# clysto/tinyimgcodec

Hardware: AMD Instinct MI355X
Metric: Mpixels/s encode (DCT+quant kernel) (higher is better)
Workload: dtype f32+f64

## Files before the change

tinyimgcodec_amd/csrc/lint_strip_kernel.py:

```python
#!/usr/bin/env python3
import os
import re
import shutil
import subprocess
import sys
import tempfile

LLVM = "/opt/rocm/lib/llvm/bin"


class ToolsMissing(RuntimeError):
    pass


def device_code_objects(lib_path, tmp):
    bundler, objdump, readelf = (os.path.join(LLVM, t) for t in ("clang-offload-bundler", "llvm-objdump", "llvm-readelf"))
    if shutil.which("objcopy") is None or not all(os.path.exists(t) for t in (bundler, objdump, readelf)):
        raise ToolsMissing("binutils / ROCm llvm tools not available")
    fat = os.path.join(tmp, "fat.bin")
    subprocess.run(["objcopy", "-O", "binary", "--only-section=.hip_fatbin", lib_path, fat], check=True)
    blob = open(fat, "rb").read()
    magic = b"__CLANG_OFFLOAD_BUNDLE__"
    starts = [i for i in range(len(blob)) if blob.startswith(magic, i)]
    out = []
    for k, st in enumerate(starts):
        part = os.path.join(tmp, "bundle%d.bin" % k)
        with open(part, "wb") as f:
            f.write(blob[st:starts[k + 1] if k + 1 < len(starts) else len(blob)])
        co = os.path.join(tmp, "dev%d.co" % k)
        subprocess.run([bundler, "--unbundle", "--type=o", "--input=" + part, "--targets=hipv4-amdgcn-amd-amdhsa--gfx950", "--output=" + co], check=True)
        out.append((co, objdump, readelf))
    return out


def check(lib_path):
    found = []
    with tempfile.TemporaryDirectory() as tmp:
        for co, objdump, readelf in device_code_objects(lib_path, tmp):
            dis = subprocess.run([objdump, "-d", "--no-show-raw-insn", co], capture_output=True, text=True, check=True).stdout
            for m in re.finditer(r"<(_ZN3tic17dctq_strip_kernel\w+)>:\n(.*?)(?=\n\n|\Z)", dis, re.S):
                name, body = m.group(1), m.group(2)
                insns = [ln.split("//")[0].strip() for ln in body.splitlines() if ln.strip()]
                reserved = re.compile(r"\bv7[2-9]\b|\bv\[(\d+):(\d+)\]")

                def touches(ins):
                    for mm in reserved.finditer(ins):
                        if mm.group(1) is None:
                            return True
                        if int(mm.group(2)) >= 72 and int(mm.group(1)) <= 79:
                            return True
                    return False

                n_loads = n_moves = n_take = n_cvt = 0
                for k, ins in enumerate(insns):
                    if not touches(ins):
                        continue
                    if re.match(r"global_load_dwordx2 v\[7[246]:7[357]\], v\d+, s\[\d+:\d+\]", ins) or re.match(r"global_load_dwordx4 v\[76:79\], v\d+, s\[\d+:\d+\]", ins):
                        n_loads += 1
                        continue
                    tk = re.match(r"ds_write_b64 v(\d+), v\[7[246]:7[357]\]$", ins)
                    cv = re.match(r"v_cvt_f32_ubyte[0-3](_e32)? v(\d+), v(7[2-9])$", ins)
                    mv = re.match(r"v_mov_b32(_e32)? v(\d+), v(7[2-9])$", ins)
                    assert (tk and int(tk.group(1)) < 72) or (cv and int(cv.group(2)) < 72) or (mv and int(mv.group(2)) < 72), "unexpected use of a reserved register: " + ins
                    prev = insns[k - 1]
                    if tk:
                        n_take += 1
                        assert prev.startswith("s_waitcnt vmcnt("), "the LDS store out of a landing pair is not behind its counted wait: %s | %s" % (prev, ins)
                    elif cv:
                        n_cvt += 1
                        assert prev.startswith("s_waitcnt vmcnt(") or re.match(r"v_cvt_f32_ubyte[0-3](_e32)? v\d+, v7[2-9]$", prev), \
                            "a conversion out of a landing register is not behind its counted wait: %s | %s" % (prev, ins)
                    else:
                        n_moves += 1
                cols = n_take > 0
                assert n_loads >= 7 and n_moves >= 4 and ((cols and n_take >= 5 and n_cvt == 0) or (not cols and n_cvt >= 24 and n_cvt % 8 == 0)), (name, n_loads, n_take, n_cvt, n_moves)
                assert "accvgpr" not in body and "scratch_" not in body, "the strip kernel uses accumulator registers or scratch"
                notes = subprocess.run([readelf, "--notes", co], capture_output=True, text=True, check=True).stdout
                blk = [e for e in notes.split("\n  - .agpr_count:") if (".name:" in e and name in e)][0]
                blk = ".agpr_count:" + blk
                assert re.search(r"\.vgpr_count:\s+80\b", blk) and re.search(r"\.private_segment_fixed_size:\s+0\b", blk) and re.search(r"\.agpr_count:\s+0\b", blk), blk
                found.append("%s: 80 VGPRs, no AGPRs, no scratch; v72..v79 named by %d loads, %d %s, %d moves only"
                             % ("columns-first" if cols else "rows-first", n_loads, n_take if cols else n_cvt, "LDS stores" if cols else "conversions", n_moves))
    if len(found) == 2:
        return "dctq_strip_kernel | " + " | ".join(found)
    raise AssertionError("both instantiations of dctq_strip_kernel expected in %s, found %d" % (lib_path, len(found)))


if __name__ == "__main__":
    try:
        print("lint_strip_kernel: " + check(sys.argv[1]))
    except ToolsMissing as e:
        sys.stderr.write("lint_strip_kernel: %s\n" % e)
        sys.exit(2)
    except AssertionError as e:
        sys.stderr.write("lint_strip_kernel FAILED: %s\n" % (e,))
        sys.exit(1)
```

tinyimgcodec_amd/csrc/tic_kernels.hip:

```cpp
#include <hip/hip_runtime.h>
#include <hip/hip_ext.h>
#include <stddef.h>
#include <stdint.h>
#include <stdlib.h>
#include <string.h>
#include <type_traits>

#include "tic_hooks.h"
#include "tic_kernels.h"
#include "tic_rd_plan.h"
#include "tic_strip_plan.h"
#include "tic_math.h"

namespace tic {

#define TIC_DPP_QP_XOR1 0xB1
#define TIC_DPP_QP_XOR2 0x4E
#define TIC_DPP_ROW_SHL4 0x104
#define TIC_DPP_ROW_SHR4 0x114

__device__ __forceinline__ uint32_t perm_b32(uint32_t hi_src, uint32_t lo_src, uint32_t sel) {
    return __builtin_amdgcn_perm(hi_src, lo_src, sel);
}

__device__ __forceinline__ void transpose8x8_bytes(uint32_t &lo, uint32_t &hi, int i) {
    uint32_t nhi = (uint32_t)__builtin_amdgcn_update_dpp((int)hi, (int)lo, TIC_DPP_ROW_SHL4, 0xf, 0x5, false);
    uint32_t nlo = (uint32_t)__builtin_amdgcn_update_dpp((int)lo, (int)hi, TIC_DPP_ROW_SHR4, 0xf, 0xa, false);
    lo = nlo;
    hi = nhi;
    uint32_t selB = (i & 2) ? 0x03020706u : 0x05040100u;
    uint32_t plo = (uint32_t)__builtin_amdgcn_mov_dpp((int)lo, TIC_DPP_QP_XOR2, 0xf, 0xf, true);
    uint32_t phi = (uint32_t)__builtin_amdgcn_mov_dpp((int)hi, TIC_DPP_QP_XOR2, 0xf, 0xf, true);
    lo = perm_b32(plo, lo, selB);
    hi = perm_b32(phi, hi, selB);
    uint32_t selC = (i & 1) ? 0x03070105u : 0x06020400u;
    plo = (uint32_t)__builtin_amdgcn_mov_dpp((int)lo, TIC_DPP_QP_XOR1, 0xf, 0xf, true);
    phi = (uint32_t)__builtin_amdgcn_mov_dpp((int)hi, TIC_DPP_QP_XOR1, 0xf, 0xf, true);
    lo = perm_b32(plo, lo, selC);
    hi = perm_b32(phi, hi, selC);
}

__device__ __forceinline__ void transpose8x8_bytes_shfl(uint32_t &lo, uint32_t &hi, int i) {
    uint32_t row[2] = {lo, hi};
    uint32_t col_lo = 0, col_hi = 0;
    int base = (threadIdx.x & 63) & ~7;
    for (int r = 0; r < 8; r++) {
        uint32_t l = __shfl(row[0], base + r, 64), h = __shfl(row[1], base + r, 64);
        uint32_t w = (i < 4) ? l : h;
        uint32_t byte = (w >> (8 * (i & 3))) & 0xffu;
        if (r < 4)
            col_lo |= byte << (8 * r);
        else
            col_hi |= byte << (8 * (r - 4));
    }
    lo = col_lo;
    hi = col_hi;
}

__device__ __forceinline__ void wave_lds_fence() {
    __builtin_amdgcn_fence(__ATOMIC_RELEASE, "wavefront");
    __builtin_amdgcn_wave_barrier();
    __builtin_amdgcn_fence(__ATOMIC_ACQUIRE, "wavefront");
}

__device__ __forceinline__ int reflect_index(int i, int n) {
    if (i < n) return i;
    if (n >= 8) return 2 * (n - 1) - i;
    if (n == 1) return 0;
    int p = 2 * (n - 1), j = i;
    while (j >= p) j -= p;
    return j < n ? j : p - j;
}

constexpr int kWavesPerWG = 4;
static_assert(kWavesPerWG == kStripWavesPerWG, "tic_strip_plan.h plans for this workgroup");
constexpr int kLdsStrideDw = 68;
constexpr int kZzStrideB = 144;
constexpr int kLdsWaveBytes = 8 * kLdsStrideDw * 4;

struct Strip {
    int by, bx;
    bool valid;
    size_t oblk;
};

__device__ __forceinline__ void load_block_row(const uint8_t *__restrict__ img, int h, int w, long stride, bool aligned8,
                                               const Strip &s, int i, uint32_t &lo, uint32_t &hi) {
    lo = 0;
    hi = 0;
    if (!s.valid) return;
    int y = reflect_index(s.by * 8 + i, h);
    int x0 = s.bx * 8;
    const uint8_t *p = img + (long)y * stride + x0;
    if (aligned8 && x0 + 8 <= w) {
        uint2 v = *reinterpret_cast<const uint2 *>(p);
        lo = v.x;
        hi = v.y;
    } else {
        const uint8_t *rowp = img + (long)y * stride;
#pragma unroll
        for (int k = 0; k < 8; k++) {
            uint32_t b = rowp[reflect_index(x0 + k, w)];
            if (k < 4)
                lo |= b << (8 * k);
            else
                hi |= b << (8 * (k - 4));
        }
    }
}

__device__ __forceinline__ void transpose8x8_dwords(uint32_t *lds, int b, int i, uint32_t v[8]) {
    uint32_t *blk = lds + b * kLdsStrideDw;
#pragma unroll
    for (int u = 0; u < 8; u++) blk[u * 8 + i] = v[u];
    wave_lds_fence();
    const uint4 *rp = reinterpret_cast<const uint4 *>(blk + i * 8);
    uint4 a = rp[0], c = rp[1];
    v[0] = a.x; v[1] = a.y; v[2] = a.z; v[3] = a.w;
    v[4] = c.x; v[5] = c.y; v[6] = c.z; v[7] = c.w;
    wave_lds_fence();
}

__device__ __forceinline__ void exact_block(uint32_t colLo, uint32_t colHi, uint32_t *lds, int b, int i,
                                         const DctqConsts *__restrict__ C, int q[8]) {
    double c[8];
#pragma unroll
    for (int r = 0; r < 4; r++) {
        c[r] = (double)((int)((colLo >> (8 * r)) & 0xffu) - 128);
        c[r + 4] = (double)((int)((colHi >> (8 * r)) & 0xffu) - 128);
    }
    dct8_exact(c[0], c[1], c[2], c[3], c[4], c[5], c[6], c[7]);
    uint32_t w[8];
#pragma unroll
    for (int k = 0; k < 8; k++) w[k] = (uint32_t)__double2loint(c[k]);
    transpose8x8_dwords(lds, b, i, w);
    uint32_t wh[8];
#pragma unroll
    for (int k = 0; k < 8; k++) wh[k] = (uint32_t)__double2hiint(c[k]);
    transpose8x8_dwords(lds, b, i, wh);
#pragma unroll
    for (int k = 0; k < 8; k++) c[k] = __hiloint2double((int)wh[k], (int)w[k]);
    dct8_exact(c[0], c[1], c[2], c[3], c[4], c[5], c[6], c[7]);
    const double *div = C->div + i * 8;
#pragma unroll
    for (int v = 0; v < 8; v++) {
        q[v] = (int)rint(c[v] / div[v]);
        __builtin_amdgcn_sched_barrier(0);
    }
}

__device__ __forceinline__ void store_zigzag(uint32_t *lds, int b, int i, const uint16_t zz[8], const int q[8],
                                             int16_t *__restrict__ out, const Strip &s) {
    char *blk = reinterpret_cast<char *>(lds) + b * kZzStrideB;
#pragma unroll
    for (int v = 0; v < 8; v++) *reinterpret_cast<int16_t *>(blk + zz[v]) = (int16_t)q[v];
    wave_lds_fence();
    uint4 val = *reinterpret_cast<const uint4 *>(blk + i * 16);
    wave_lds_fence();
    if (s.valid) *reinterpret_cast<uint4 *>(out + s.oblk * 64 + i * 8) = val;
}

__device__ __forceinline__ Strip make_strip(int tile, int ntiles, int tiles_x, int bw, int b) {
    Strip s;
    int ty = tile / tiles_x;
    int tx = tile - ty * tiles_x;
    s.by = ty;
    s.bx = tx * 8 + b;
    s.valid = (tile < ntiles) && (s.bx < bw);
    s.oblk = (size_t)ty * bw + s.bx;
    return s;
}

__global__ __launch_bounds__(kWavesPerWG * 64) void dctq_exact_kernel(DctqArgs a) {
    __shared__ __attribute__((aligned(16))) uint32_t lds_all[kWavesPerWG][kLdsWaveBytes / 4];
    a.img += (long)blockIdx.y * a.frame_stride_in;
    a.out = reinterpret_cast<int16_t *>(reinterpret_cast<char *>(a.out) + (long)blockIdx.y * a.frame_stride_out);
    const int lane = threadIdx.x & 63, wave = threadIdx.x >> 6;
    const int b = lane >> 3, i = lane & 7;
    uint32_t *lds = lds_all[wave];
    int tile = blockIdx.x * kWavesPerWG + wave;
    int ntiles = a.ntiles;
    if (a.rem_mode) {
        const int bh = a.ntiles / a.tiles_x, rw = a.tiles_x - a.fast_tx;
        const int n_right = bh * rw, n_bottom = (bh - a.fast_ty) * a.fast_tx;
        ntiles = 0;
        if (tile < n_right) {
            tile = (tile / rw) * a.tiles_x + a.fast_tx + tile % rw;
            ntiles = a.ntiles;
        } else if (tile < n_right + n_bottom) {
            const int k = tile - n_right;
            tile = (a.fast_ty + k / a.fast_tx) * a.tiles_x + k % a.fast_tx;
            ntiles = a.ntiles;
        }
    }
    Strip s = make_strip(tile, ntiles, a.tiles_x, a.bw, b);
    uint32_t lo, hi;
    load_block_row(a.img, a.h, a.w, a.stride, a.aligned8, s, i, lo, hi);
    transpose8x8_bytes(lo, hi, i);
    int q[8];
    exact_block(lo, hi, lds, b, i, a.consts, q);
    const uint4 zzv = *reinterpret_cast<const uint4 *>(a.consts->zzofs + i * 8);
    uint16_t zz[8] = {(uint16_t)zzv.x, (uint16_t)(zzv.x >> 16), (uint16_t)zzv.y, (uint16_t)(zzv.y >> 16),
                      (uint16_t)zzv.z, (uint16_t)(zzv.z >> 16), (uint16_t)zzv.w, (uint16_t)(zzv.w >> 16)};
    store_zigzag(lds, b, i, zz, q, a.out, s);
}

constexpr int kTWaveBytes = kLdsWaveBytes;
constexpr int kTHalfDw = 272;
constexpr int kZzWaveBytes = 8 * kZzStrideB;
constexpr int kPxBlkBytes = 80;
constexpr int kChunkStrips = 8;

__device__ __forceinline__ void quant_fma(float z, float mul, uint32_t &bits, float &d) {
    const float s = fmaf(z, mul, kMagic);
    bits = __float_as_uint(s);
    const float nr = kMagic - s;
    d = fmaf(z, mul, nr);
}

__device__ __forceinline__ void store16_wt_nt(void *p, const uint4 &v) {
    typedef uint32_t u32x4 __attribute__((ext_vector_type(4)));
    const u32x4 d = {v.x, v.y, v.z, v.w};
    asm volatile("global_store_dwordx4 %0, %1, off sc1 nt" : : "v"(p), "v"(d) : "memory");
}
__device__ __forceinline__ void store16_wt_nt(const void *sbase, uint32_t voff, const uint4 &v) {
    typedef uint32_t u32x4 __attribute__((ext_vector_type(4)));
    const u32x4 d = {v.x, v.y, v.z, v.w};
    asm volatile("global_store_dwordx4 %0, %1, %2 sc1 nt" : : "v"(voff), "v"(d), "s"(sbase) : "memory");
}

constexpr int kBatch = 8;
constexpr int kBatchWaveBytes = kBatch * (128 + 64) + 64;

template <int CTRL>
__device__ __forceinline__ double dpp_f64(double x) {
    const int lo = __builtin_amdgcn_mov_dpp(__double2loint(x), CTRL, 0xf, 0xf, true);
    const int hi = __builtin_amdgcn_mov_dpp(__double2hiint(x), CTRL, 0xf, 0xf, true);
    return __hiloint2double(hi, lo);
}

__device__ __forceinline__ int rational_quad(const uint32_t *ldsT, int b, int i, const double *cst_rat) {
#pragma clang fp contract(off)
    const int w = i >> 2, k = i & 3;
    const uint32_t ca = (0x05010300u >> (8 * k)) & 0xffu, cb = (0x06020407u >> (8 * k)) & 0xffu;
    const uint32_t *row = ldsT + w * 128 + 4 * b;
    const float fa = __uint_as_float(row[(ca >> 2) * kTHalfDw + (ca & 3)]);
    const float fb = __uint_as_float(row[(cb >> 2) * kTHalfDw + (cb & 3)]);
    const double K = w ? (kTW3 * 0.5) : (kSq2h * 0.5);
    const double ya = (double)fa * K, yb = (double)fb * K;
    const double p = ya + yb;
    const double s2 = p + dpp_f64<TIC_DPP_QP_XOR1>(p);
    const double o = dpp_f64<TIC_DPP_QP_XOR2>(s2);
    const double E = (k & 1) ? s2 - o : s2 + o;
    const double X = E * ((k & 1) ? (kTW3 * 0.5) : (kSq2h * 0.5));
    const double div = cst_rat[2 * w + (k & 1)], rdiv = cst_rat[4 + 2 * w + (k & 1)];
    return (int)rint(div_rn(X, div, rdiv));
}

__device__ __forceinline__ int rational_slim(uint32_t rowLo, uint32_t rowHi, int i, const double *cst_rat) {
#pragma clang fp contract(off)
    uint32_t lo = perm_b32(rowHi, rowLo, 0x04030700u);
    uint32_t hi = perm_b32(rowHi, rowLo, 0x06050201u);
    transpose8x8_bytes(lo, hi, i);
    const uint32_t tot = __builtin_amdgcn_sad_u8(lo, 0u, __builtin_amdgcn_sad_u8(hi, 0u, 0u));
    const uint32_t sa = __builtin_amdgcn_sad_u8(lo & 0xff0000ffu, 0u, __builtin_amdgcn_sad_u8(hi & 0xff0000ffu, 0u, 0u));
    const int e0 = (int)tot - 1024, e4 = 2 * (int)sa - (int)tot;
    double y0 = (double)e0 * (kSq2h * 0.5);
    double y4 = (double)e4 * (kTW3 * 0.5);
    y0 = y0 + dpp_f64<TIC_DPP_QP_XOR1>(y0);
    y4 = y4 + dpp_f64<TIC_DPP_QP_XOR1>(y4);
    y0 = y0 + dpp_f64<TIC_DPP_QP_XOR2>(y0);
    y4 = y4 + dpp_f64<TIC_DPP_QP_XOR2>(y4);
    const double b0 = dpp_f64<TIC_DPP_ROW_SHL4>(y0), b4 = dpp_f64<TIC_DPP_ROW_SHL4>(y4);
    const double A = (i & 2) ? y4 : y0, B = (i & 2) ? b4 : b0;
    const double E = (i & 1) ? A - B : A + B;
    const double X = E * ((i & 1) ? (kTW3 * 0.5) : (kSq2h * 0.5));
    const double div = cst_rat[i & 3], rdiv = cst_rat[4 + (i & 3)];
    return (int)rint(div_rn(X, div, rdiv));
}
__device__ __forceinline__ unsigned long long wave_redo_block(const uint8_t *px , double *tbuf ,
                                                              const double *cosm, const double *rdiv, const uint16_t *zzofs, int16_t *img16,
                                                              int lane) {
    const int u = lane >> 3, c = lane & 7;
    typedef double d2 __attribute__((ext_vector_type(2)));
    const d2 *mu = reinterpret_cast<const d2 *>(cosm + u * 8), *mc = reinterpret_cast<const d2 *>(cosm + c * 8);
    const d2 m0 = mu[0], m1 = mu[1], m2 = mu[2], m3 = mu[3];
    double x[8];
#pragma unroll
    for (int r = 0; r < 8; r++) x[r] = (double)((int)px[r * 8 + c] - 128);
    double ta = m0.x * x[0], tb = m0.y * x[1];
    ta = fma(m1.x, x[2], ta); tb = fma(m1.y, x[3], tb);
    ta = fma(m2.x, x[4], ta); tb = fma(m2.y, x[5], tb);
    ta = fma(m3.x, x[6], ta); tb = fma(m3.y, x[7], tb);
    tbuf[u * 8 + c] = ta + tb;
    const d2 n0 = mc[0], n1 = mc[1], n2 = mc[2], n3 = mc[3];
    wave_lds_fence();
    const d2 *tu = reinterpret_cast<const d2 *>(tbuf + u * 8);
    const d2 y0 = tu[0], y1 = tu[1], y2 = tu[2], y3 = tu[3];
    double xa = n0.x * y0.x, xb = n0.y * y0.y;
    xa = fma(n1.x, y1.x, xa); xb = fma(n1.y, y1.y, xb);
    xa = fma(n2.x, y2.x, xa); xb = fma(n2.y, y2.y, xb);
    xa = fma(n3.x, y3.x, xa); xb = fma(n3.y, y3.y, xb);
    const double X = xa + xb;
    const double tq = X * rdiv[lane], rq = rint(tq);
    const bool rational = (lane & 0x1b) == 0;
    const bool decided = fabs(tq - rq) < 0.5 - 1e-9;
    if (decided && !rational) img16[zzofs[lane] >> 1] = (int16_t)(int)rq;
    const unsigned long long und = __ballot(!decided && !rational);
    wave_lds_fence();
    return und;
}

__device__ __forceinline__ uint32_t second_level_8(uint32_t colLo, uint32_t colHi, uint32_t *lds, int b, int i, const double *mul64, int q[8]) {
    double c[8];
#pragma unroll
    for (int r = 0; r < 4; r++) {
        c[r] = (double)(int)((colLo >> (8 * r)) & 0xffu);
        c[r + 4] = (double)(int)((colHi >> (8 * r)) & 0xffu);
    }
    dct8_aan(c[0], c[1], c[2], c[3], c[4], c[5], c[6], c[7]);
    c[0] -= 1024.0;
    uint32_t w[8], wh[8];
#pragma unroll
    for (int k = 0; k < 8; k++) w[k] = (uint32_t)__double2loint(c[k]);
    transpose8x8_dwords(lds, b, i, w);
#pragma unroll
    for (int k = 0; k < 8; k++) wh[k] = (uint32_t)__double2hiint(c[k]);
    transpose8x8_dwords(lds, b, i, wh);
#pragma unroll
    for (int k = 0; k < 8; k++) c[k] = __hiloint2double((int)wh[k], (int)w[k]);
    dct8_aan(c[0], c[1], c[2], c[3], c[4], c[5], c[6], c[7]);
    uint32_t und = 0;
#pragma unroll
    for (int v = 0; v < 8; v++) {
        const double t = c[v] * mul64[i * 8 + v], r = rint(t);
        q[v] = (int)r;
        if (!(fabs(t - r) < 0.5 - 1e-9)) und |= 1u << v;
    }
    return und;
}

struct StripKernargs {
    const uint8_t *img;
    const DctqConsts *consts;
    StripHead hd;
    StripWarm w;
    DctqArgs a;
};
static_assert(offsetof(StripKernargs, hd) == 16 && sizeof(StripHead) == 40 && offsetof(StripKernargs, w) == 64, "leading scalars, then one line");

template <class T>
__device__ __forceinline__ uint32_t lds_addr(T *p) {
    return (uint32_t)(uintptr_t)(__attribute__((address_space(3))) char *)(p);
}
template <class T>
__device__ __forceinline__ T *lds_ptr(uint32_t v) {
    return (T *)(__attribute__((address_space(3))) T *)(uintptr_t)v;
}

template <bool kCols>
__global__ __launch_bounds__(kWavesPerWG * 64, 6) __attribute__((amdgpu_num_vgpr(72))) void dctq_strip_kernel(
    const uint8_t *img, const DctqConsts *consts, unsigned long long hd_split, uint32_t hd_stride, uint32_t hd_misc, uint32_t hd_tstep,
    uint32_t hd_nfast, uint32_t hd_fast_tx, uint32_t hd_magic_fast_tx, uint32_t hd_in_step32, uint32_t hd_step_tx, StripWarm w, DctqArgs a) {
    const StripHead hd = {hd_split, hd_stride, hd_misc, hd_tstep, hd_nfast, hd_fast_tx, hd_magic_fast_tx, hd_in_step32, hd_step_tx};
    __shared__ __attribute__((aligned(16))) uint32_t ldsT_all[kWavesPerWG][kTWaveBytes / 4];
    __shared__ __attribute__((aligned(16))) uint32_t ldsZ_all[kWavesPerWG][kZzWaveBytes / 4];
    __shared__ __attribute__((aligned(16))) unsigned char cst_blk[kStripBlkBytes];
    __shared__ __attribute__((aligned(16))) uint32_t bat_all[kWavesPerWG][kBatchWaveBytes / 4];
    const int lane = threadIdx.x & 63;
    const int wave = __builtin_amdgcn_readfirstlane(threadIdx.x >> 6);
    uint32_t *ldsT = ldsT_all[wave];
    char *ldsZ = reinterpret_cast<char *>(ldsZ_all[wave]);
    const uint16_t *cst_zz = reinterpret_cast<const uint16_t *>(cst_blk + kBlkZz);
    const double *cst_rat = reinterpret_cast<const double *>(cst_blk + kBlkRat);
    uint4 *bat_img = reinterpret_cast<uint4 *>(bat_all[wave]);
    uint2 *bat_pix = reinterpret_cast<uint2 *>(bat_all[wave] + kBatch * 32);
    uint32_t *bat_id = bat_all[wave] + kBatch * 48;
    const DctqConsts *__restrict__ C = consts;
    const uint8_t *img_s = img;
    if (__builtin_expect(blockIdx.z != 0, 0)) {
        asm volatile("" : : : "memory");
        img_s += (long)blockIdx.z * w.frame_stride_in;
    }

    const int lr = lane >> 3, lb = lane & 7;
    const int b = lane >> 3, i = lane & 7;
    unsigned long long mask_exact = 0;
    uint32_t n_second = 0, n_quad = 0;
    int nE = 0;
    int t_first, n_my;
    int16_t *out_f;
    uint32_t st_off = (uint32_t)lane * 16u;
    {
        typedef float f32x4 __attribute__((ext_vector_type(4)));
        typedef uint32_t u32x4 __attribute__((ext_vector_type(4)));
        f32x4 m0, m1;
        f32x4 thr;
        u32x4 zzv;
        u32x4 c_fill;
        {
            constexpr int kPpw = kStripBlkPieces / kWavesPerWG;
            static_assert(kPpw * kWavesPerWG == kStripBlkPieces && kPpw <= 64, "constant block must split evenly over the waves");
            const uint32_t piece = lane < kPpw ? (uint32_t)(wave * kPpw + lane) : (uint32_t)kStripBlkPieces - 1u;
            const uint32_t fo = piece * 16u;
            asm volatile("global_load_dwordx4 v[76:79], %0, %1" : : "v"(fo), "s"(C->strip_blk) : "memory", "v76", "v77", "v78", "v79");
        }
        const uint32_t ld_off = (uint32_t)lr * hd.stride + (uint32_t)lb * 8u;

        const StripCursor cur = strip_cursor(hd, w, blockIdx.x, blockIdx.y, (uint32_t)wave);
        n_my = cur.n_my;
        t_first = (int)cur.t_first;
        uint32_t txp = cur.txp, in_off = cur.in_off, oblk;
        const uint32_t in_wrap32 = strip_in_wrap(hd);
        uint32_t src_off = 0;
        int n_issued = 0;
#define TIC_RSV_CLOBBER "memory", "v72", "v73", "v74", "v75", "v76", "v77", "v78", "v79"
#define TIC_LOAD(R, OB)                                                                                      \
    do {                                                                                                     \
        src_off = n_issued < n_my ? in_off : src_off;                                                        \
        OB = oblk;                                                                                           \
        asm volatile("global_load_dwordx2 v[" R "], %0, %1" : : "v"(ld_off), "s"(img_s + src_off) : TIC_RSV_CLOBBER); \
        n_issued++;                                                                                          \
        strip_step(txp, in_off, oblk, hd.step_tx, hd.fast_tx, hd.in_step32, in_wrap32, w);                   \
    } while (0)
#define TIC_LOAD_HEAD(R, WRAP)                                                                               \
    do {                                                                                                     \
        src_off = n_issued < n_my ? in_off : src_off;                                                        \
        asm volatile("global_load_dwordx2 v[" R "], %0, %1" : : "v"(ld_off), "s"(img_s + src_off) : TIC_RSV_CLOBBER); \
        n_issued++;                                                                                          \
        WRAP = strip_step_in(txp, in_off, hd.step_tx, hd.fast_tx, hd.in_step32, in_wrap32);                  \
    } while (0)
#define TIC_TAKE_COLS(R, N) asm volatile("s_waitcnt vmcnt(" #N ")\n\tds_write_b64 %0, v[" R "]" : : "v"(px_wr) : TIC_RSV_CLOBBER)
#define TIC_TAKE_ROWS(D, R0, R1, N)                                                                          \
    asm volatile("s_waitcnt vmcnt(" #N ")\n\tv_cvt_f32_ubyte0 %0, v" #R0 "\n\tv_cvt_f32_ubyte1 %1, v" #R0 "\n\tv_cvt_f32_ubyte2 %2, v" #R0 \
                 "\n\tv_cvt_f32_ubyte3 %3, v" #R0 "\n\tv_cvt_f32_ubyte0 %4, v" #R1 "\n\tv_cvt_f32_ubyte1 %5, v" #R1                       \
                 "\n\tv_cvt_f32_ubyte2 %6, v" #R1 "\n\tv_cvt_f32_ubyte3 %7, v" #R1                                                       \
                 : "=v"(D[0]), "=v"(D[1]), "=v"(D[2]), "=v"(D[3]), "=v"(D[4]), "=v"(D[5]), "=v"(D[6]), "=v"(D[7]) : : TIC_RSV_CLOBBER)
        uint32_t ob0, ob1, ob2;
        uint32_t kstrip = 0;
        bool wrap0, wrap1;
        uint32_t ty0 = cur.ty, tx0 = cur.txp;
        TIC_LOAD_HEAD("72:73", wrap0);
        TIC_LOAD_HEAD("74:75", wrap1);
        asm volatile("; block indices: behind the loads" : "+s"(ty0), "+s"(tx0) : "s"(w.round_wgs), "s"(w.round_span), "s"(w.magic_round_wgs) : TIC_RSV_CLOBBER);
        oblk = strip_oblk(ty0, tx0, w);
        ob0 = oblk;
        strip_step_blk(oblk, wrap0, w);
        ob1 = oblk;
        strip_step_blk(oblk, wrap1, w);
        constexpr int kHalf = kCols ? kTHalfDw : 256;
        const int p1a = kCols ? i : lr, p1b = kCols ? b : lb;
        uint32_t px_wr = lds_addr(ldsZ + lb * kPxBlkBytes + lr * 8);
        uint32_t o_px_rd = lds_addr(ldsZ + b * kPxBlkBytes + i);
        uint32_t o_twA = lds_addr(ldsT + (p1a >> 2) * kHalf + (p1a & 3) + 4 * p1b);
        uint32_t o_twB = lds_addr(ldsT + (p1a >> 2) * kHalf + (p1a & 3) + 4 * (p1b ^ 4));
        uint32_t q_tr = (uint32_t)(i * 8 + (b ^ (4 * ((i >> 1) & 1))));
        uint32_t q_zr = (uint32_t)(i * 8 + (b ^ (kCols ? (((i >> 1) & 1) | (i & 4)) : (4 * ((i >> 1) & 1)))));
        uint32_t o_zb = lds_addr(ldsZ);
        asm volatile("; addresses of the loop" : "+v"(px_wr), "+v"(o_px_rd), "+v"(o_twA), "+v"(o_twB), "+v"(q_tr), "+v"(q_zr), "+v"(o_zb), "+v"(st_off) : : TIC_RSV_CLOBBER);
        const uint8_t *px_rd = lds_ptr<const uint8_t>(o_px_rd);
        uint32_t *twA = lds_ptr<uint32_t>(o_twA), *twB = lds_ptr<uint32_t>(o_twB);
        const uint4 *tr = reinterpret_cast<const uint4 *>(__builtin_assume_aligned(ldsT, 16)) + q_tr;
        const uint4 *zr = reinterpret_cast<const uint4 *>(__builtin_assume_aligned(ldsZ, 16)) + q_zr;
        char *zb = lds_ptr<char>(o_zb);
        out_f = reinterpret_cast<int16_t *>(reinterpret_cast<char *>(w.out) + (long)blockIdx.z * w.frame_stride_out);
        asm volatile("s_waitcnt vmcnt(2)\n\tv_mov_b32 %0, v76\n\tv_mov_b32 %1, v77\n\tv_mov_b32 %2, v78\n\tv_mov_b32 %3, v79"
                     : "=v"(c_fill.x), "=v"(c_fill.y), "=v"(c_fill.z), "=v"(c_fill.w) : : "memory", "v76", "v77", "v78", "v79");
        if (lane < kStripBlkPieces / kWavesPerWG) *reinterpret_cast<u32x4 *>(cst_blk + (wave * (kStripBlkPieces / kWavesPerWG) + lane) * 16) = c_fill;
        asm volatile("s_waitcnt lgkmcnt(0)\n\ts_barrier" : : : "memory");
        m0 = *reinterpret_cast<const f32x4 *>(cst_blk + (kCols ? kBlkMul : kBlkMulT) + i * 32);
        m1 = *reinterpret_cast<const f32x4 *>(cst_blk + (kCols ? kBlkMul : kBlkMulT) + i * 32 + 16);
        thr = *reinterpret_cast<const f32x4 *>(cst_blk + (kCols ? kBlkThr : kBlkThrT) + i * 16);
        zzv = *reinterpret_cast<const u32x4 *>(cst_blk + (kCols ? kBlkZz : kBlkZzT) + i * 16);
        auto zz_ptr = [&](uint32_t ofs) {
            const uint32_t c = ofs >> 4;
            return reinterpret_cast<int16_t *>(zb + c * 128 + (ofs & 15) + 16 * (b ^ (kCols ? (((c >> 1) & 1) | (c & 4)) : (4 * ((c >> 1) & 1)))));
        };
        int16_t *zp0 = zz_ptr(zzv.x & 0xffff), *zp1 = zz_ptr(zzv.x >> 16), *zp2 = zz_ptr(zzv.y & 0xffff), *zp3 = zz_ptr(zzv.y >> 16);
        int16_t *zp4 = zz_ptr(zzv.z & 0xffff), *zp5 = zz_ptr(zzv.z >> 16), *zp6 = zz_ptr(zzv.w & 0xffff), *zp7 = zz_ptr(zzv.w >> 16);
        wave_lds_fence();

        int left = n_my;
        auto raw_words = [&](auto tag, uint32_t &lo, uint32_t &hi) {
            constexpr int R = decltype(tag)::value;
            static_assert(R == 72 || R == 74 || R == 76, "landing register pair");
            if constexpr (R == 72) asm volatile("v_mov_b32 %0, v72\n\tv_mov_b32 %1, v73" : "=v"(lo), "=v"(hi) : : "memory");
            else if constexpr (R == 74) asm volatile("v_mov_b32 %0, v74\n\tv_mov_b32 %1, v75" : "=v"(lo), "=v"(hi) : : "memory");
            else asm volatile("v_mov_b32 %0, v76\n\tv_mov_b32 %1, v77" : "=v"(lo), "=v"(hi) : : "memory");
        };
        auto process = [&](auto tag, const float (&pxr)[8], const uint32_t ob) {
            float d0, d1, d2, d3, d4, d5, d6, d7;
            if constexpr (kCols) {
                d0 = (float)px_rd[0]; d1 = (float)px_rd[8]; d2 = (float)px_rd[16]; d3 = (float)px_rd[24];
                d4 = (float)px_rd[32]; d5 = (float)px_rd[40]; d6 = (float)px_rd[48]; d7 = (float)px_rd[56];
            } else {
                d0 = pxr[0]; d1 = pxr[1]; d2 = pxr[2]; d3 = pxr[3]; d4 = pxr[4]; d5 = pxr[5]; d6 = pxr[6]; d7 = pxr[7];
            }
            dct8_aan(d0, d1, d2, d3, d4, d5, d6, d7);
            d0 -= 1024.0f;
            twA[0 * 32] = __float_as_uint(d0); twA[1 * 32] = __float_as_uint(d1); twB[2 * 32] = __float_as_uint(d2);
            twB[3 * 32] = __float_as_uint(d3); twA[4 * 32] = __float_as_uint(d4); twA[5 * 32] = __float_as_uint(d5);
            twB[6 * 32] = __float_as_uint(d6); twB[7 * 32] = __float_as_uint(d7);
            wave_lds_fence();
            const uint4 ra = tr[0], rb = tr[kHalf / 4];
            wave_lds_fence();
            float e0 = __uint_as_float(ra.x), e1 = __uint_as_float(ra.y), e2 = __uint_as_float(ra.z), e3 = __uint_as_float(ra.w);
            float e4 = __uint_as_float(rb.x), e5 = __uint_as_float(rb.y), e6 = __uint_as_float(rb.z), e7 = __uint_as_float(rb.w);
            dct8_aan(e0, e1, e2, e3, e4, e5, e6, e7);
            uint32_t q0, q1, q2, q3, q4, q5, q6, q7;
            float r0, r1, r2, r3, r4, r5, r6, r7;
            quant_fma(e0, m0.x, q0, r0); quant_fma(e1, m0.y, q1, r1); quant_fma(e2, m0.z, q2, r2); quant_fma(e3, m0.w, q3, r3);
            quant_fma(e4, m1.x, q4, r4); quant_fma(e5, m1.y, q5, r5); quant_fma(e6, m1.z, q6, r6); quant_fma(e7, m1.w, q7, r7);
            const float mA1 = fmaxf(fmaxf(fabsf(r1), fabsf(r2)), fabsf(r3));
            const float mA2 = fmaxf(fmaxf(fabsf(r5), fabsf(r6)), fabsf(r7));
            const float mB = fmaxf(fabsf(r0), fabsf(r4));
            const unsigned long long cA = __ballot(mA1 > thr.x) | __ballot(mA2 > thr.y);
            const unsigned long long cB = __ballot(mB > thr.z);
            *zp0 = (int16_t)q0; *zp1 = (int16_t)q1; *zp2 = (int16_t)q2; *zp3 = (int16_t)q3;
            *zp4 = (int16_t)q4; *zp5 = (int16_t)q5; *zp6 = (int16_t)q6; *zp7 = (int16_t)q7;
            const unsigned long long kRat = 0x1111111111111111ull;
            if (__builtin_expect((cB & kRat) != 0ull, 0)) {
                n_quad++;
                if constexpr (kCols) {
                    const int rq = rational_quad(ldsT, b, i, cst_rat);
                    if ((i & 2) == 0) *zz_ptr(28u * (uint32_t)(i & 1) + 20u * (uint32_t)(i >> 2) + 30u * (uint32_t)((i & 1) & (i >> 2))) = (int16_t)rq;
                } else {
                    uint32_t lo0, hi0;
                    raw_words(tag, lo0, hi0);
                    uint2 *pb = reinterpret_cast<uint2 *>(ldsT);
                    pb[lb * 8 + lr] = make_uint2(lo0, hi0);
                    wave_lds_fence();
                    const uint2 rowv = pb[lane];
                    wave_lds_fence();
                    const int rq = rational_slim(rowv.x, rowv.y, i, cst_rat);
                    if (i < 4) *zz_ptr(i == 0 ? 0u : (i == 1 ? 28u : (i == 2 ? 20u : 78u))) = (int16_t)rq;
                }
            }
            wave_lds_fence();
            const uint4 val = *zr;
            wave_lds_fence();
            const char *dst = reinterpret_cast<const char *>(out_f) + ((unsigned long long)ob << 7);
            const unsigned long long mG = cA | (cB & ~kRat);
            if (__builtin_expect(mG != 0ull, 0)) {
                const uint32_t gm = (uint32_t)__ballot(((mG >> (8u * (uint32_t)i)) & 0xffull) != 0ull) & 0xffu;
                const int nnew = __builtin_popcount(gm);
                if (nE + nnew <= kBatch && gm != 0xffu) {
                    uint32_t lo0, hi0;
                    raw_words(tag, lo0, hi0);
                    const uint32_t below = (1u << b) - 1u, lbelow = (1u << lb) - 1u;
                    const bool mine = (gm >> b) & 1u;
                    const int e = nE + __builtin_popcount(gm & below);
                    if (mine) bat_img[e * 8 + i] = val;
                    if (mine && i == 0) bat_id[e] = ob + (uint32_t)b;
                    if ((gm >> lb) & 1u) bat_pix[(nE + __builtin_popcount(gm & lbelow)) * 8 + lr] = make_uint2(lo0, hi0);
                    if (!mine) store16_wt_nt(dst, st_off, val);
                    nE += nnew;
                    n_second += (uint32_t)nnew;
                } else {
                    mask_exact |= 1ull << kstrip;
                    store16_wt_nt(dst, st_off, val);
                }
            } else
                store16_wt_nt(dst, st_off, val);
            left--;
            kstrip++;
        };
        float pxf[8] = {0.f, 0.f, 0.f, 0.f, 0.f, 0.f, 0.f, 0.f};
#define TIC_STEP(RLOAD, OBL, RTAKE, R0, R1, OBP, N)                                                          \
        TIC_LOAD(RLOAD, OBL);                                                                                \
        if constexpr (kCols) { TIC_TAKE_COLS(RTAKE, N); } else { TIC_TAKE_ROWS(pxf, R0, R1, N); }            \
        process(std::integral_constant<int, R0>(), pxf, OBP)
        do {
            if (left == 0) break;
            TIC_STEP("76:77", ob2, "72:73", 72, 73, ob0, 2);
            if (left == 0) break;
            TIC_STEP("72:73", ob0, "74:75", 74, 75, ob1, 3);
            while (left != 0) {
                TIC_STEP("74:75", ob1, "76:77", 76, 77, ob2, 4);
                if (left == 0) break;
                TIC_STEP("76:77", ob2, "72:73", 72, 73, ob0, 4);
                if (left == 0) break;
                TIC_STEP("72:73", ob0, "74:75", 74, 75, ob1, 4);
            }
        } while (0);
#undef TIC_STEP
        asm volatile("; end of the strip walk" : : : TIC_RSV_CLOBBER);
#undef TIC_LOAD
#undef TIC_LOAD_HEAD
#undef TIC_TAKE_COLS
#undef TIC_TAKE_ROWS
#undef TIC_RSV_CLOBBER
    }
    typedef const __attribute__((address_space(4))) char *kernarg_ptr;
    kernarg_ptr kargs = (kernarg_ptr)__builtin_amdgcn_kernarg_segment_ptr();
    asm volatile("; rare paths: DctqArgs from here on" : "+s"(kargs));
    const __attribute__((address_space(4))) DctqArgs *ca = reinterpret_cast<const __attribute__((address_space(4))) DctqArgs *>(kargs + offsetof(StripKernargs, a));
    (void)a;
    if (nE != 0) {
        const double *cst_cos = reinterpret_cast<const double *>(cst_blk + kBlkCos);
        const double *cst_rdiv = reinterpret_cast<const double *>(cst_blk + kBlkRdiv);
        uint32_t m_exact = 0;
        if (nE < 3) {
            for (int ee = 0; ee < nE; ee++) {
                const unsigned long long und = wave_redo_block(reinterpret_cast<const uint8_t *>(bat_pix + ee * 8), reinterpret_cast<double *>(ldsT), cst_cos,
                                                               cst_rdiv, cst_zz, reinterpret_cast<int16_t *>(bat_img + ee * 8), lane);
                if (und != 0ull) m_exact |= 1u << ee;
            }
        } else {
            const bool have2 = b < nE;
            const int e2 = have2 ? b : 0;
            const uint2 rowv = bat_pix[e2 * 8 + i];
            uint32_t lo = rowv.x, hi = rowv.y;
            transpose8x8_bytes(lo, hi, i);
            int qs[8];
            uint32_t und = second_level_8(lo, hi, ldsT, b, i, reinterpret_cast<const double *>(cst_blk + kBlkMul64), qs);
            if ((i & 3) == 0) und &= ~0x11u;
            const uint4 zo = *reinterpret_cast<const uint4 *>(cst_zz + i * 8);
            const uint32_t zw[4] = {zo.x, zo.y, zo.z, zo.w};
            int16_t *img2 = reinterpret_cast<int16_t *>(bat_img + e2 * 8);
            if (have2) {
#pragma unroll
                for (int v = 0; v < 8; v++)
                    if (!((und >> v) & 1u) && !((i & 3) == 0 && (v & 3) == 0)) img2[((zw[v >> 1] >> (16 * (v & 1))) & 0xffffu) >> 1] = (int16_t)qs[v];
            }
            const unsigned long long um = __ballot(have2 && und != 0u);
            for (int ee = 0; ee < nE; ee++)
                if ((um >> (8 * ee)) & 0xffull) m_exact |= 1u << ee;
        }
        const bool have = b < nE;
        const int e = have ? b : 0;
        const uint32_t blk = bat_id[e];
        if (m_exact != 0u) {
            const uint2 rowv = bat_pix[e * 8 + i];
            int16_t *img16 = reinterpret_cast<int16_t *>(bat_img + e * 8);
            uint32_t lo = rowv.x, hi = rowv.y;
            transpose8x8_bytes(lo, hi, i);
            const uint4 zo = *reinterpret_cast<const uint4 *>(cst_zz + i * 8);
            const uint32_t zw[4] = {zo.x, zo.y, zo.z, zo.w};
            int qx[8];
            exact_block(lo, hi, ldsT, b, i, C, qx);
            if (have && ((m_exact >> e) & 1u)) {
#pragma unroll
                for (int v = 0; v < 8; v++) img16[((zw[v >> 1] >> (16 * (v & 1))) & 0xffffu) >> 1] = (int16_t)qx[v];
            }
        }
        wave_lds_fence();
        const uint4 val = bat_img[e * 8 + i];
        if (have) store16_wt_nt(reinterpret_cast<char *>(out_f) + ((unsigned long long)blk << 7) + (uint32_t)i * 16u, val);
    }
    if (ca->fallback_count != nullptr && lane == 0) {
        if (n_second != 0) atomicAdd(ca->fallback_count, (unsigned long long)n_second);
        if (n_quad != 0) atomicAdd(ca->fallback_count + 1, (unsigned long long)n_quad);
        if (mask_exact != 0ull) atomicAdd(ca->fallback_count + 2, (unsigned long long)__builtin_popcountll(mask_exact));
        if (nE != 0) atomicMax(ca->fallback_count + 3, (unsigned long long)nE);
    }
    if (mask_exact == 0ull) return;
    asm volatile("s_waitcnt vmcnt(0)" : : : "memory");
    const uint4 zzn = *reinterpret_cast<const uint4 *>(cst_zz + i * 8);
    const uint16_t zz[8] = {(uint16_t)zzn.x, (uint16_t)(zzn.x >> 16), (uint16_t)zzn.y, (uint16_t)(zzn.y >> 16),
                            (uint16_t)zzn.z, (uint16_t)(zzn.z >> 16), (uint16_t)zzn.w, (uint16_t)(zzn.w >> 16)};
    for (unsigned long long todo = mask_exact; todo != 0ull; todo &= todo - 1ull) {
        const int k = __builtin_ctzll(todo);
        const long t = (long)t_first + (long)k * ca->tstep;
        const int ty = (int)(t / ca->fast_tx), tx = (int)(t - (long)ty * ca->fast_tx);
        Strip s;
        s.by = ty;
        s.bx = tx * 8 + b;
        s.valid = true;
        s.oblk = (size_t)ty * ca->bw + s.bx;
        uint32_t lo, hi;
        load_block_row(img_s, ca->h, ca->w, ca->stride, true, s, i, lo, hi);
        transpose8x8_bytes(lo, hi, i);
        int q[8];
        const uint32_t und = second_level_8(lo, hi, ldsT, b, i, reinterpret_cast<const double *>(cst_blk + kBlkMul64), q);
        if (__ballot(und != 0u) != 0ull) exact_block(lo, hi, ldsT, b, i, C, q);
        store_zigzag(reinterpret_cast<uint32_t *>(ldsZ), b, i, zz, q, out_f, s);
    }
}

__global__ __launch_bounds__(kWavesPerWG * 64) void dctq_exact_wide_kernel(WideArgs a) {
    __shared__ __attribute__((aligned(16))) uint32_t lds_all[kWavesPerWG][kLdsWaveBytes / 4];
    const int lane = threadIdx.x & 63, wave = threadIdx.x >> 6;
    const int b = lane >> 3, i = lane & 7;
    uint32_t *lds = lds_all[wave];
    const int tile = blockIdx.x * kWavesPerWG + wave;
    Strip s = make_strip(tile, a.ntiles, a.tiles_x, a.bw, b);
    double c[8];
#pragma unroll
    for (int r = 0; r < 8; r++) c[r] = 0.0;
    if (s.valid) {
        const int x = reflect_index(s.bx * 8 + i, a.w);
#pragma unroll
        for (int r = 0; r < 8; r++) {
            const int y = reflect_index(s.by * 8 + r, a.h);
            c[r] = (double)a.img[(long)y * a.stride + x] - 128.0;
        }
    }
    dct8_exact(c[0], c[1], c[2], c[3], c[4], c[5], c[6], c[7]);
    uint32_t w[8], wh[8];
#pragma unroll
    for (int k = 0; k < 8; k++) w[k] = (uint32_t)__double2loint(c[k]);
    transpose8x8_dwords(lds, b, i, w);
#pragma unroll
    for (int k = 0; k < 8; k++) wh[k] = (uint32_t)__double2hiint(c[k]);
    transpose8x8_dwords(lds, b, i, wh);
#pragma unroll
    for (int k = 0; k < 8; k++) c[k] = __hiloint2double((int)wh[k], (int)w[k]);
    dct8_exact(c[0], c[1], c[2], c[3], c[4], c[5], c[6], c[7]);
    if (!s.valid) return;
    const double *div = a.consts->div + i * 8;
    const uint16_t *zz = a.consts->zzofs + i * 8;
    int32_t *ob = a.out + s.oblk * 64;
#pragma unroll
    for (int v = 0; v < 8; v++) {
        ob[zz[v] >> 1] = (int32_t)rint(c[v] / div[v]);
        __builtin_amdgcn_sched_barrier(0);
    }
}

__constant__ int kAnnScalesInt[64] = {
    16384, 22725, 21407, 19266, 16384, 12873, 8867,  4520,  22725, 31521, 29692, 26722, 22725, 17855, 12299, 6270,
    21407, 29692, 27969, 25172, 21407, 16819, 11585, 5906,  19266, 26722, 25172, 22654, 19266, 15137, 10426, 5315,
    16384, 22725, 21407, 19266, 16384, 12873, 8867,  4520,  12873, 17855, 16819, 15137, 12873, 10114, 6967,  3552,
    8867,  12299, 11585, 10426, 8867,  6967,  4799,  2446,  4520,  6270,  5906,  5315,  4520,  3552,  2446,  1247};

#define TIC_GLOBAL __attribute__((address_space(1)))
typedef uint32_t tic_u32x2 __attribute__((ext_vector_type(2)));
typedef uint32_t tic_u32x4 __attribute__((ext_vector_type(4)));

struct SseAcc {
    unsigned long long sq = 0, sw = 0;
};

__device__ __forceinline__ void sse_accumulate_tile(const Strip &s, int i, int h, int w, const SseArgs &m, const uint32_t px[8], SseAcc &acc) {
    uint32_t sq = 0, sw = 0;
    const int y = s.by * 8 + i, x0 = s.bx * 8;
    if (s.valid && y < h) {
        const TIC_GLOBAL uint8_t *p = (const TIC_GLOBAL uint8_t *)m.img + (long)y * m.stride + x0;
        uint32_t lo = 0, hi = 0;
        if (m.aligned8 && x0 + 8 <= w) {
            const tic_u32x2 v = *(const TIC_GLOBAL tic_u32x2 *)p;
            lo = v.x;
// ... 343 lines not shown
```

Before: 1.682 million.

## Stage column-first transpose and zig-zag through lane-linear LDS planes

For the columns-first instantiation, the per-lane scattered LDS stores of DCT rows and quantized coefficients are replaced with ds_write_addtid_b32 runs into padded planes addressed through m0. A precomputed gather table in LDS then assembles the zig-zag output from those planes. The aim is fewer LDS address computations, fewer live address registers, and fewer bank conflicts during the transpose and zig-zag staging. The cost is inline asm that writes m0 and a more complex gather readback of eight 16-bit loads per output. The lint script gains checks that m0 is set only directly in front of these store runs.

```diff
diff --git a/tinyimgcodec_amd/csrc/lint_strip_kernel.py b/tinyimgcodec_amd/csrc/lint_strip_kernel.py
--- a/tinyimgcodec_amd/csrc/lint_strip_kernel.py
+++ b/tinyimgcodec_amd/csrc/lint_strip_kernel.py
@@ -73,14 +73,37 @@
                     else:
                         n_moves += 1
                 cols = n_take > 0
+                n_m0 = n_addtid = n_run = 0
+                RUNS = (8, 4)
+                for k, ins in enumerate(insns):
+                    assert not re.match(r"(s_movrel|v_movrel|ds_gws|s_sendmsg|ds_read_addtid|global_load_lds|scratch_load_lds|s_set_gpr_idx)", ins) \
+                        and not re.match(r"buffer_load\w* .*\blds\b", ins), "an implicit reader of m0: " + ins
+                    if re.search(r"\bm0\b", ins):
+                        assert re.match(r"s_mov_b32 m0, s\d+$", ins), "m0 named outside the hand-written store statement: " + ins
+                        run = []
+                        while re.match(r"ds_write_addtid_b32 v\d+( offset:(0x[0-9a-f]+|\d+))?$", insns[k + 2 + len(run)]):
+                            run.append(insns[k + 2 + len(run)])
+                        assert insns[k + 1] == "s_nop 0" and len(run) in RUNS, \
+                            "m0 is not set directly in front of its lane-linear stores: " + " | ".join(insns[k + 1:k + 11])
+                        assert not any(touches(r) for r in run), "a lane-linear store out of a reserved register: " + " | ".join(run)
+                        n_m0 += 1
+                        n_run += len(run)
+                    elif ins.startswith("ds_write_addtid_b32"):
+                        n_addtid += 1
+                        back = insns[max(0, k - 9):k]
+                        sets = [j for j, r in enumerate(back) if r.startswith("s_mov_b32 m0,")]
+                        assert sets and all(r.startswith("ds_write_addtid_b32") or r == "s_nop 0" for r in back[sets[-1] + 1:]), \
+                            "a lane-linear store that does not follow its own write of m0: " + " | ".join(back + [ins])
+                assert n_addtid == n_run and ((cols and n_m0 >= 10 and n_run == 6 * n_m0) or (not cols and n_m0 == 0)), (name, n_m0, n_addtid)
                 assert n_loads >= 7 and n_moves >= 4 and ((cols and n_take >= 5 and n_cvt == 0) or (not cols and n_cvt >= 24 and n_cvt % 8 == 0)), (name, n_loads, n_take, n_cvt, n_moves)
                 assert "accvgpr" not in body and "scratch_" not in body, "the strip kernel uses accumulator registers or scratch"
                 notes = subprocess.run([readelf, "--notes", co], capture_output=True, text=True, check=True).stdout
                 blk = [e for e in notes.split("\n  - .agpr_count:") if (".name:" in e and name in e)][0]
                 blk = ".agpr_count:" + blk
                 assert re.search(r"\.vgpr_count:\s+80\b", blk) and re.search(r"\.private_segment_fixed_size:\s+0\b", blk) and re.search(r"\.agpr_count:\s+0\b", blk), blk
-                found.append("%s: 80 VGPRs, no AGPRs, no scratch; v72..v79 named by %d loads, %d %s, %d moves only"
-                             % ("columns-first" if cols else "rows-first", n_loads, n_take if cols else n_cvt, "LDS stores" if cols else "conversions", n_moves))
+                found.append("%s: 80 VGPRs, no AGPRs, no scratch; v72..v79 named by %d loads, %d %s, %d moves only; m0 %s"
+                             % ("columns-first" if cols else "rows-first", n_loads, n_take if cols else n_cvt, "LDS stores" if cols else "conversions", n_moves,
+                                "set %d times, each directly in front of its lane-linear stores (%d)" % (n_m0, n_run) if cols else "untouched"))
     if len(found) == 2:
         return "dctq_strip_kernel | " + " | ".join(found)
     raise AssertionError("both instantiations of dctq_strip_kernel expected in %s, found %d" % (lib_path, len(found)))
diff --git a/tinyimgcodec_amd/csrc/tic_kernels.hip b/tinyimgcodec_amd/csrc/tic_kernels.hip
--- a/tinyimgcodec_amd/csrc/tic_kernels.hip
+++ b/tinyimgcodec_amd/csrc/tic_kernels.hip
@@ -10,6 +10,7 @@
 #include "tic_kernels.h"
 #include "tic_rd_plan.h"
 #include "tic_strip_plan.h"
+#include "tic_strip_lds.h"
 #include "tic_math.h"
 
 namespace tic {
@@ -205,9 +206,10 @@
     store_zigzag(lds, b, i, zz, q, a.out, s);
 }
 
-constexpr int kTWaveBytes = kLdsWaveBytes;
-constexpr int kTHalfDw = 272;
+constexpr int kTWaveBytes = kTPlaneWaveBytes;
+static_assert(kTWaveBytes >= kLdsWaveBytes && kTWaveBytes % 16 == 0, "transpose8x8_dwords keeps its own layout in the same buffer");
 constexpr int kZzWaveBytes = 8 * kZzStrideB;
+static_assert(kZPlaneWaveBytes <= kZzWaveBytes, "the staging planes fit the zig-zag buffer");
 constexpr int kPxBlkBytes = 80;
 constexpr int kChunkStrips = 8;
 
@@ -243,9 +245,9 @@
 #pragma clang fp contract(off)
     const int w = i >> 2, k = i & 3;
     const uint32_t ca = (0x05010300u >> (8 * k)) & 0xffu, cb = (0x06020407u >> (8 * k)) & 0xffu;
-    const uint32_t *row = ldsT + w * 128 + 4 * b;
-    const float fa = __uint_as_float(row[(ca >> 2) * kTHalfDw + (ca & 3)]);
-    const float fb = __uint_as_float(row[(cb >> 2) * kTHalfDw + (cb & 3)]);
+    const uint32_t *row = ldsT + w * (4 * kTPlaneQ[4]) + 8 * b;
+    const float fa = __uint_as_float(row[ca]);
+    const float fb = __uint_as_float(row[cb]);
     const double K = w ? (kTW3 * 0.5) : (kSq2h * 0.5);
     const double ya = (double)fa * K, yb = (double)fb * K;
     const double p = ya + yb;
@@ -431,6 +433,18 @@
         WRAP = strip_step_in(txp, in_off, hd.step_tx, hd.fast_tx, hd.in_step32, in_wrap32);                  \
     } while (0)
 #define TIC_TAKE_COLS(R, N) asm volatile("s_waitcnt vmcnt(" #N ")\n\tds_write_b64 %0, v[" R "]" : : "v"(px_wr) : TIC_RSV_CLOBBER)
+#define TIC_PUT_PLANES(D0, D1, D2, D3, D4, D5, D6, D7)                                                                            \
+    asm volatile("s_mov_b32 m0, %8\n\ts_nop 0\n\tds_write_addtid_b32 %0 offset:%9\n\tds_write_addtid_b32 %1 offset:%10\n\t"         \
+                 "ds_write_addtid_b32 %2 offset:%11\n\tds_write_addtid_b32 %3 offset:%12\n\tds_write_addtid_b32 %4 offset:%13\n\t" \
+                 "ds_write_addtid_b32 %5 offset:%14\n\tds_write_addtid_b32 %6 offset:%15\n\tds_write_addtid_b32 %7 offset:%16"     \
+                 : : "v"(D0), "v"(D1), "v"(D2), "v"(D3), "v"(D4), "v"(D5), "v"(D6), "v"(D7), "s"(t_base),                          \
+                     "n"(16 * kTPlaneQ[0]), "n"(16 * kTPlaneQ[1]), "n"(16 * kTPlaneQ[2]), "n"(16 * kTPlaneQ[3]),                   \
+                     "n"(16 * kTPlaneQ[4]), "n"(16 * kTPlaneQ[5]), "n"(16 * kTPlaneQ[6]), "n"(16 * kTPlaneQ[7]) : TIC_RSV_CLOBBER)
+#define TIC_PUT_ZPLANES(W0, W1, W2, W3)                                                                                           \
+    asm volatile("s_mov_b32 m0, %4\n\ts_nop 0\n\tds_write_addtid_b32 %0 offset:%5\n\tds_write_addtid_b32 %1 offset:%6\n\t"          \
+                 "ds_write_addtid_b32 %2 offset:%7\n\tds_write_addtid_b32 %3 offset:%8"                                            \
+                 : : "v"(W0), "v"(W1), "v"(W2), "v"(W3), "s"(z_base),                                                              \
+                     "n"(4 * kZPlaneDw[0]), "n"(4 * kZPlaneDw[1]), "n"(4 * kZPlaneDw[2]), "n"(4 * kZPlaneDw[3]) : TIC_RSV_CLOBBER)
 #define TIC_TAKE_ROWS(D, R0, R1, N)                                                                          \
     asm volatile("s_waitcnt vmcnt(" #N ")\n\tv_cvt_f32_ubyte0 %0, v" #R0 "\n\tv_cvt_f32_ubyte1 %1, v" #R0 "\n\tv_cvt_f32_ubyte2 %2, v" #R0 \
                  "\n\tv_cvt_f32_ubyte3 %3, v" #R0 "\n\tv_cvt_f32_ubyte0 %4, v" #R1 "\n\tv_cvt_f32_ubyte1 %5, v" #R1                       \
@@ -448,16 +462,21 @@
         strip_step_blk(oblk, wrap0, w);
         ob1 = oblk;
         strip_step_blk(oblk, wrap1, w);
-        constexpr int kHalf = kCols ? kTHalfDw : 256;
-        const int p1a = kCols ? i : lr, p1b = kCols ? b : lb;
+        constexpr int kHalf = 256;
         uint32_t px_wr = lds_addr(ldsZ + lb * kPxBlkBytes + lr * 8);
         uint32_t o_px_rd = lds_addr(ldsZ + b * kPxBlkBytes + i);
-        uint32_t o_twA = lds_addr(ldsT + (p1a >> 2) * kHalf + (p1a & 3) + 4 * p1b);
-        uint32_t o_twB = lds_addr(ldsT + (p1a >> 2) * kHalf + (p1a & 3) + 4 * (p1b ^ 4));
-        uint32_t q_tr = (uint32_t)(i * 8 + (b ^ (4 * ((i >> 1) & 1))));
-        uint32_t q_zr = (uint32_t)(i * 8 + (b ^ (kCols ? (((i >> 1) & 1) | (i & 4)) : (4 * ((i >> 1) & 1)))));
+        uint32_t o_twA = lds_addr(ldsT + (lr >> 2) * kHalf + (lr & 3) + 4 * lb);
+        uint32_t o_twB = lds_addr(ldsT + (lr >> 2) * kHalf + (lr & 3) + 4 * (lb ^ 4));
+        const uint32_t t_base = lds_addr(ldsT);
+        uint32_t q_tr = kCols ? (uint32_t)(kTPlaneStepQ * (i >> 1) + kTPlaneOddQ * (i & 1) + 2 * b)
+                              : (uint32_t)(i * 8 + (b ^ (4 * ((i >> 1) & 1))));
+        uint32_t q_zr = (uint32_t)(i * 8 + (b ^ (4 * ((i >> 1) & 1))));
         uint32_t o_zb = lds_addr(ldsZ);
-        asm volatile("; addresses of the loop" : "+v"(px_wr), "+v"(o_px_rd), "+v"(o_twA), "+v"(o_twB), "+v"(q_tr), "+v"(q_zr), "+v"(o_zb), "+v"(st_off) : : TIC_RSV_CLOBBER);
+        const uint32_t z_base = lds_addr(ldsZ);
+        if constexpr (kCols)
+            asm volatile("; addresses of the loop" : "+v"(px_wr), "+v"(o_px_rd), "+v"(q_tr), "+v"(o_zb), "+v"(st_off) : : TIC_RSV_CLOBBER);
+        else
+            asm volatile("; addresses of the loop" : "+v"(px_wr), "+v"(o_px_rd), "+v"(o_twA), "+v"(o_twB), "+v"(q_tr), "+v"(q_zr), "+v"(o_zb), "+v"(st_off) : : TIC_RSV_CLOBBER);
         const uint8_t *px_rd = lds_ptr<const uint8_t>(o_px_rd);
         uint32_t *twA = lds_ptr<uint32_t>(o_twA), *twB = lds_ptr<uint32_t>(o_twB);
         const uint4 *tr = reinterpret_cast<const uint4 *>(__builtin_assume_aligned(ldsT, 16)) + q_tr;
@@ -474,11 +493,25 @@
         zzv = *reinterpret_cast<const u32x4 *>(cst_blk + (kCols ? kBlkZz : kBlkZzT) + i * 16);
         auto zz_ptr = [&](uint32_t ofs) {
             const uint32_t c = ofs >> 4;
-            return reinterpret_cast<int16_t *>(zb + c * 128 + (ofs & 15) + 16 * (b ^ (kCols ? (((c >> 1) & 1) | (c & 4)) : (4 * ((c >> 1) & 1)))));
+            return reinterpret_cast<int16_t *>(zb + c * 128 + (ofs & 15) + 16 * (b ^ (4 * ((c >> 1) & 1))));
         };
         int16_t *zp0 = zz_ptr(zzv.x & 0xffff), *zp1 = zz_ptr(zzv.x >> 16), *zp2 = zz_ptr(zzv.y & 0xffff), *zp3 = zz_ptr(zzv.y >> 16);
         int16_t *zp4 = zz_ptr(zzv.z & 0xffff), *zp5 = zz_ptr(zzv.z >> 16), *zp6 = zz_ptr(zzv.w & 0xffff), *zp7 = zz_ptr(zzv.w >> 16);
         wave_lds_fence();
+        const uint16_t *zg0 = nullptr, *zg1 = nullptr, *zg2 = nullptr, *zg3 = nullptr, *zg4 = nullptr, *zg5 = nullptr, *zg6 = nullptr, *zg7 = nullptr;
+        if constexpr (kCols) {
+            char *inv = reinterpret_cast<char *>(ldsT);
+            auto put = [&](uint32_t ofs, int v) { *reinterpret_cast<uint16_t *>(inv + ofs) = (uint16_t)(strip_zstage_byte(0, v) + 4 * i); };
+            put(zzv.x & 0xffff, 0); put(zzv.x >> 16, 1); put(zzv.y & 0xffff, 2); put(zzv.y >> 16, 3);
+            put(zzv.z & 0xffff, 4); put(zzv.z >> 16, 5); put(zzv.w & 0xffff, 6); put(zzv.w >> 16, 7);
+            wave_lds_fence();
+            const uint4 gv = reinterpret_cast<const uint4 *>(__builtin_assume_aligned(ldsT, 16))[i];
+            wave_lds_fence();
+            const char *gb = zb + 32 * b;
+            auto at = [&](uint32_t ofs) { return reinterpret_cast<const uint16_t *>(gb + ofs); };
+            zg0 = at(gv.x & 0xffff); zg1 = at(gv.x >> 16); zg2 = at(gv.y & 0xffff); zg3 = at(gv.y >> 16);
+            zg4 = at(gv.z & 0xffff); zg5 = at(gv.z >> 16); zg6 = at(gv.w & 0xffff); zg7 = at(gv.w >> 16);
+        }
 
         int left = n_my;
         auto raw_words = [&](auto tag, uint32_t &lo, uint32_t &hi) {
@@ -498,11 +531,15 @@
             }
             dct8_aan(d0, d1, d2, d3, d4, d5, d6, d7);
             d0 -= 1024.0f;
-            twA[0 * 32] = __float_as_uint(d0); twA[1 * 32] = __float_as_uint(d1); twB[2 * 32] = __float_as_uint(d2);
-            twB[3 * 32] = __float_as_uint(d3); twA[4 * 32] = __float_as_uint(d4); twA[5 * 32] = __float_as_uint(d5);
-            twB[6 * 32] = __float_as_uint(d6); twB[7 * 32] = __float_as_uint(d7);
+            if constexpr (kCols) {
+                TIC_PUT_PLANES(d0, d1, d2, d3, d4, d5, d6, d7);
+            } else {
+                twA[0 * 32] = __float_as_uint(d0); twA[1 * 32] = __float_as_uint(d1); twB[2 * 32] = __float_as_uint(d2);
+                twB[3 * 32] = __float_as_uint(d3); twA[4 * 32] = __float_as_uint(d4); twA[5 * 32] = __float_as_uint(d5);
+                twB[6 * 32] = __float_as_uint(d6); twB[7 * 32] = __float_as_uint(d7);
+            }
             wave_lds_fence();
-            const uint4 ra = tr[0], rb = tr[kHalf / 4];
+            const uint4 ra = tr[0], rb = tr[kCols ? 1 : kHalf / 4];
             wave_lds_fence();
             float e0 = __uint_as_float(ra.x), e1 = __uint_as_float(ra.y), e2 = __uint_as_float(ra.z), e3 = __uint_as_float(ra.w);
             float e4 = __uint_as_float(rb.x), e5 = __uint_as_float(rb.y), e6 = __uint_as_float(rb.z), e7 = __uint_as_float(rb.w);
@@ -516,14 +553,22 @@
             const float mB = fmaxf(fabsf(r0), fabsf(r4));
             const unsigned long long cA = __ballot(mA1 > thr.x) | __ballot(mA2 > thr.y);
             const unsigned long long cB = __ballot(mB > thr.z);
-            *zp0 = (int16_t)q0; *zp1 = (int16_t)q1; *zp2 = (int16_t)q2; *zp3 = (int16_t)q3;
-            *zp4 = (int16_t)q4; *zp5 = (int16_t)q5; *zp6 = (int16_t)q6; *zp7 = (int16_t)q7;
+            if constexpr (kCols) {
+                const uint32_t qq[8] = {q0, q1, q2, q3, q4, q5, q6, q7};
+                const uint32_t w0 = perm_b32(qq[kZPairHi[0]], qq[kZPairLo[0]], 0x05040100u), w1 = perm_b32(qq[kZPairHi[1]], qq[kZPairLo[1]], 0x05040100u);
+                const uint32_t w2 = perm_b32(qq[kZPairHi[2]], qq[kZPairLo[2]], 0x05040100u), w3 = perm_b32(qq[kZPairHi[3]], qq[kZPairLo[3]], 0x05040100u);
+                TIC_PUT_ZPLANES(w0, w1, w2, w3);
+            } else {
+                *zp0 = (int16_t)q0; *zp1 = (int16_t)q1; *zp2 = (int16_t)q2; *zp3 = (int16_t)q3;
+                *zp4 = (int16_t)q4; *zp5 = (int16_t)q5; *zp6 = (int16_t)q6; *zp7 = (int16_t)q7;
+            }
             const unsigned long long kRat = 0x1111111111111111ull;
             if (__builtin_expect((cB & kRat) != 0ull, 0)) {
                 n_quad++;
                 if constexpr (kCols) {
                     const int rq = rational_quad(ldsT, b, i, cst_rat);
-                    if ((i & 2) == 0) *zz_ptr(28u * (uint32_t)(i & 1) + 20u * (uint32_t)(i >> 2) + 30u * (uint32_t)((i & 1) & (i >> 2))) = (int16_t)rq;
+                    constexpr int kV0 = strip_zstage_byte(0, 0), kV4 = strip_zstage_byte(0, 4);
+                    if ((i & 2) == 0) *reinterpret_cast<int16_t *>(zb + kV0 + (kV4 - kV0) * (i & 1) + 16 * (i >> 2) + 32 * b) = (int16_t)rq;
                 } else {
                     uint32_t lo0, hi0;
                     raw_words(tag, lo0, hi0);
@@ -537,7 +582,12 @@
                 }
             }
             wave_lds_fence();
-            const uint4 val = *zr;
+            uint4 val;
+            if constexpr (kCols) {
+                const uint32_t h0 = *zg0, h1 = *zg1, h2 = *zg2, h3 = *zg3, h4 = *zg4, h5 = *zg5, h6 = *zg6, h7 = *zg7;
+                val = make_uint4(h0 | (h1 << 16), h2 | (h3 << 16), h4 | (h5 << 16), h6 | (h7 << 16));
+            } else
+                val = *zr;
             wave_lds_fence();
             const char *dst = reinterpret_cast<const char *>(out_f) + ((unsigned long long)ob << 7);
             const unsigned long long mG = cA | (cB & ~kRat);
@@ -588,6 +638,8 @@
 #undef TIC_LOAD
 #undef TIC_LOAD_HEAD
 #undef TIC_TAKE_COLS
+#undef TIC_PUT_PLANES
+#undef TIC_PUT_ZPLANES
 #undef TIC_TAKE_ROWS
 #undef TIC_RSV_CLOBBER
     }
diff --git a/tinyimgcodec_amd/csrc/tic_strip_lds.h b/tinyimgcodec_amd/csrc/tic_strip_lds.h
--- /dev/null
+++ b/tinyimgcodec_amd/csrc/tic_strip_lds.h
@@ -0,0 +1,32 @@
+#pragma once
+
+namespace tic {
+
+constexpr int kTPlaneQ[8] = {0, 17, 40, 57, 80, 97, 120, 137};
+constexpr int kTPlaneStepQ = 40;
+constexpr int kTPlaneOddQ = 17;
+constexpr int kTPlaneWaveBytes = 2448;
+
+constexpr bool strip_tplanes_ok() {
+    for (int u = 0; u < 8; u++)
+        if (kTPlaneQ[u] != kTPlaneStepQ * (u >> 1) + kTPlaneOddQ * (u & 1) || (kTPlaneQ[u] + 16) * 16 > kTPlaneWaveBytes) return false;
+    return kTPlaneQ[0] == 0;
+}
+static_assert(strip_tplanes_ok(), "plane table, lane formula and buffer size must agree");
+
+constexpr int kZPlaneDw[4] = {0, 64, 135, 199};
+constexpr int kZPairLo[4] = {0, 1, 2, 4};
+constexpr int kZPairHi[4] = {5, 3, 7, 6};
+constexpr int kZPlaneWaveBytes = 1052;
+constexpr int kZGatherConflictCycles = 8;
+
+constexpr int strip_zstage_byte(int u, int v) {
+    for (int p = 0; p < 4; p++) {
+        if (kZPairLo[p] == v) return 4 * kZPlaneDw[p] + 4 * u;
+        if (kZPairHi[p] == v) return 4 * kZPlaneDw[p] + 4 * u + 2;
+    }
+    return -1;
+}
+static_assert(strip_zstage_byte(7, 6) == 4 * 199 + 28 + 2 && strip_zstage_byte(0, 0) == 0, "every v has its plane and half");
+
+}
```

Result: faster. 1.726 million (median of 6 runs) (+2.6%).
